# zoj613/OccuSpytial

Hardware: AMD Instinct MI355X
Metric: Gibbs iterations/sec on 100x100 ICAR lattice, 4 chains; 1/2/4/8 GPUs (higher is better)
Workload: dtype f64; 1 GPU; 100x100 queen ICAR lattice, 10000 sites, 5 visits/site, p=q=2, 4 chains per GPU batched in every kernel (BASELINE configs[1] data, the metric's 4 chains); chains_per_gpu=4, total_chains=4, sites=10000, visit_rows=50000, parallelism=chains sharded 4/GPU, no data-path collective; one GPU, communicator=single process, problem_transport=none, krylov_cap=0, stalls=0, solve_form=k_iter, one XCD per chain, solve_workgroups_per_chain=23, main_stream_cus=160, fused_fallbacks=0, threads_per_block=64

## Files before the change

occuspytial_amd/csrc/occ_kernels.hpp:

```cpp
#pragma once
#include <float.h>
#include <hip/hip_runtime.h>
#include <stdint.h>

#include "occ_plan.hpp"
#include "occ_rng.hpp"
#include "occ_state.hpp"

namespace occ {


#ifndef OCC_SLOT_ALIGN
#define OCC_SLOT_ALIGN 8
#endif
struct alignas(OCC_SLOT_ALIGN) Slot {
    double beta1, beta, oldb, alfa, dbar, epsln, phibar, rhs1, rhs2, tnorm2, gmax, gmin, cs, sn, root;
    double ibeta;
    int itn;
    int istop;
    int done;
    int pad;
};

#define OCC_SLOT_FIELDS(X) \
// ... 450 lines not shown
    for (int k = 0; k < D; ++k) {
        const double e = normal(k);
#pragma unroll
        for (int i = k; i < D; ++i) o[i] += U[k][i] * e;
    }
#pragma unroll
    for (int i = 0; i < D; ++i) o[i] += r[i];
#pragma unroll
    for (int i = 0; i < D; ++i) {
        double v = o[i];
#pragma unroll
        for (int k = 0; k < i; ++k) v -= U[k][i] * o[k];
        o[i] = v / U[i][i];
    }
#pragma unroll
    for (int i = D - 1; i >= 0; --i) {
        double v = o[i];
#pragma unroll
        for (int k = i + 1; k < D; ++k) v -= U[i][k] * o[k];
        o[i] = v / U[i][i];
    }
#pragma unroll
    for (int i = 0; i < D; ++i) out[i] = o[i];
    return ok;
}

template <int D>
__device__ __forceinline__ bool precision_mvnorm_reg(const double (&acc)[nacc(D)], const double *prec0, const double *pbm,
                                                     uint64_t key, uint32_t it, uint32_t stream, double (&out)[D],
                                                     const double *eps_inj = nullptr)
{
    return precision_mvnorm_with<D>(acc, prec0, pbm, out,
                                    [=](int k) { return eps_inj ? eps_inj[k] : block_normal(key, (uint32_t)k, 0, it, stream); });
}


enum : int { SYNC_MAIN = 0, SYNC_ALPHA = 16, SYNC_NOISE = 32, SYNC_MAIN_SEQ = 48, SYNC_SIDE_SEQ = 52, SYNC_ABORT = 56, SYNC_DEBUG = 57, SYNC_WORDS = 64 };
constexpr unsigned SYNC_SPIN_LIMIT = 1u << 19;

__device__ __forceinline__ unsigned sync_read(const unsigned *p)
{
    return __hip_atomic_load(p, __ATOMIC_RELAXED, __HIP_MEMORY_SCOPE_AGENT);
}
__device__ __forceinline__ void sync_set(unsigned *p, unsigned v)
{
    __hip_atomic_store(p, v, __ATOMIC_RELAXED, __HIP_MEMORY_SCOPE_AGENT);
}
__device__ __forceinline__ bool sync_wait(unsigned *sync, int word, unsigned target)
{
    unsigned spins = 0;
    while ((int)(sync_read(sync + word) - target) < 0) {
        __builtin_amdgcn_s_sleep(4);
        ++spins;
        if ((spins & 63u) == 0u && sync_read(sync + SYNC_ABORT) != 0u) return false;
        if (spins > SYNC_SPIN_LIMIT) {
            sync_set(sync + SYNC_ABORT, 1u);
            return false;
        }
    }
    return true;
}
__device__ __forceinline__ double load_agent(const double *p)
{
    return __hip_atomic_load(p, __ATOMIC_RELAXED, __HIP_MEMORY_SCOPE_AGENT);
}
__device__ __forceinline__ uint64_t uniform_u64(uint64_t v)
{
    const unsigned lo = (unsigned)__builtin_amdgcn_readfirstlane((int)(unsigned)v), hi = (unsigned)__builtin_amdgcn_readfirstlane((int)(unsigned)(v >> 32));
    return ((uint64_t)hi << 32) | lo;
}
__device__ __forceinline__ double uniform_f64(double v) { return __longlong_as_double((long long)uniform_u64((uint64_t)__double_as_longlong(v))); }

__global__ void __launch_bounds__(64) k_stream_probe_wait(unsigned *w)
{
    if (threadIdx.x != 0) return;
    unsigned seen = 0u, spins = 0u;
    for (; spins < (1u << 13); ++spins) {
        if (sync_read(w) != 0u) { seen = 1u; break; }
        __builtin_amdgcn_s_sleep(16);
    }
    w[16] = seen;
    w[17] = spins;
}
__global__ void __launch_bounds__(64) k_stream_probe_set(unsigned *w)
{
    if (threadIdx.x == 0) sync_set(w, 1u);
}

__global__ void __launch_bounds__(256) k_checksum(const unsigned char *__restrict__ data, unsigned long long bytes, unsigned long long *__restrict__ out)
{
    const unsigned long long nw = (bytes + 7ull) / 8ull;
    unsigned long long acc = 0ull;
    for (unsigned long long i = (unsigned long long)blockIdx.x * blockDim.x + threadIdx.x; i < nw; i += (unsigned long long)gridDim.x * blockDim.x) {
        unsigned long long w = 0ull;
        if (8ull * i + 8ull <= bytes) w = *reinterpret_cast<const unsigned long long *>(data + 8ull * i);
        else
            for (unsigned long long b = 8ull * i; b < bytes; ++b) w |= (unsigned long long)data[b] << (8ull * (b - 8ull * i));
        unsigned long long x = w + 0x9E3779B97F4A7C15ull * (i + 1ull);
        x = (x ^ (x >> 30)) * 0xBF58476D1CE4E5B9ull;
        x = (x ^ (x >> 27)) * 0x94D049BB133111EBull;
        acc += x ^ (x >> 31);
    }
    atomicAdd(out, acc);
}

__global__ void __launch_bounds__(256) k_snapshot(const double *__restrict__ eta, double *__restrict__ s_eta, const uint8_t *__restrict__ z, uint8_t *__restrict__ s_z,
                                                  const double2 *__restrict__ x, double2 *__restrict__ s_x, unsigned long long count,
                                                  const double *__restrict__ theta, double *__restrict__ s_theta, unsigned long long count_theta,
                                                  unsigned long long *__restrict__ clock,
                                                  ChainScalars *__restrict__ scs, int n_chains, int parity, uint32_t n_iter, uint32_t burnin, uint32_t keep)
{
    if (clock != nullptr && blockIdx.x == 0 && threadIdx.x < 4) clock[threadIdx.x] = threadIdx.x == 0 ? ~0ull : 0ull;
    if (scs != nullptr && blockIdx.x == 0) {
        for (int ch = (int)threadIdx.x; ch < n_chains; ch += (int)blockDim.x) {
            ChainScalars &sc = scs[ch];
            Ctl &ctl = sc.ctl[parity];
            sc.it_base = ctl.it;
            sc.it_stop = ctl.it + n_iter;
            sc.burnin = burnin;
            sc.keep = keep;
            ctl.koff = 0;
        }
    }
    for (unsigned long long i = (unsigned long long)blockIdx.x * blockDim.x + threadIdx.x; i < count; i += (unsigned long long)gridDim.x * blockDim.x) {
        s_eta[i] = eta[i];
        s_z[i] = z[i];
        s_x[i] = x[i];
    }
    for (unsigned long long i = (unsigned long long)blockIdx.x * blockDim.x + threadIdx.x; i < count_theta; i += (unsigned long long)gridDim.x * blockDim.x) s_theta[i] = theta[i];
}

__global__ void __launch_bounds__(64) k_gate(const Ctx *__restrict__ cp, ChainScalars *__restrict__ scs)
{
    const Ctx &c = *cp;
    if (c.sync == nullptr || threadIdx.x != 0) return;
    const unsigned j = c.sync[SYNC_SIDE_SEQ];
    if (c.sync[SYNC_DEBUG] != 0u) return;
    sync_set(c.sync + SYNC_NOISE, j);
    if (!sync_wait(c.sync, SYNC_MAIN, j)) scs[0].err = -2;
}

#define OCC_KARGS const Ctx *__restrict__ cp, ChainScalars *__restrict__ scs, Slot *__restrict__ slots, int chain_base, int e

__device__ __forceinline__ double quad_site(const Ctx &c, const double *eta, int i, double eta_i)
{
    const int lane = i & 63;
    int base, width;
    slice_of(c, i, base, width);
    double qe = c.qdiag[i] * eta_i;
    for (int k = 0; k < width; ++k) qe = fma(c.sell_val[base + k * 64 + lane], eta[c.sell_col[base + k * 64 + lane]], qe);
    return eta_i * qe;
}

template <int P>
__device__ __forceinline__ void omega_b_body(const Ctx &c, uint64_t key, const double (&beta)[P], int chain, uint32_t it, int blk,
                                             bool per_wave = false)
{
    const int n = c.n;
    const double *eta = c.eta + (size_t)chain * n;
    double om = 0.0;
    {
        const int i = blk * blockDim.x + threadIdx.x;
        if (i < n) {
            double xb = 0.0;
#pragma unroll
            for (int a = 0; a < P; ++a) xb += c.Xt[(size_t)a * n + i] * beta[a];
            om = pg1_draw(key, (uint32_t)i, it, STREAM_OMEGA_B, xb + eta[i]);
        }
    }
    int t = (int)threadIdx.x;
    asm volatile("" : "+v"(t));
    const int i = blk * (int)blockDim.x + t;
    double quad[1] = {0.0};
    if (i < n) {
        c.omega_b[it & 1][(size_t)chain * n + i] = om;
        quad[0] = quad_site(c, eta, i, eta[i]);
    }
    if (per_wave) {
        const double t = wave_sum(quad[0]);
        const int slice = blk * (int)(blockDim.x >> 6) + (int)(threadIdx.x >> 6);
        if ((threadIdx.x & 63) == 0 && slice < c.nb_n) c.part_quad[(size_t)chain * c.nb_n + slice] = t;
        return;
    }
    block_partials<1>(quad, c.part_quad + (size_t)chain * c.nb_n, c.nb_n, blk);
}

__device__ __forceinline__ void omega_b_body_g(const Ctx &c, const ChainScalars &sc, int chain, uint32_t it, int blk, bool per_wave = false)
{
    const int n = c.n, i = blk * blockDim.x + threadIdx.x;
    double quad[1] = {0.0};
    if (i < n) {
        const size_t ci = (size_t)chain * n + i;
        const double *eta = c.eta + (size_t)chain * n;
        double xb = 0.0;
        for (int a = 0; a < c.p; ++a) xb += c.Xt[(size_t)a * n + i] * sc.beta[a];
        const double eta_i = eta[i];
        c.omega_b[it & 1][ci] = pg1_draw(sc.key, (uint32_t)i, it, STREAM_OMEGA_B, xb + eta_i);
        quad[0] = quad_site(c, eta, i, eta_i);
    }
    if (per_wave) {
        const double t = wave_sum(quad[0]);
        const int slice = blk * (int)(blockDim.x >> 6) + (int)(threadIdx.x >> 6);
        if ((threadIdx.x & 63) == 0 && slice < c.nb_n) c.part_quad[(size_t)chain * c.nb_n + slice] = t;
        return;
    }
    block_partials<1>(quad, c.part_quad + (size_t)chain * c.nb_n, c.nb_n, blk);
}

template <int P>
__global__ void __launch_bounds__(256) k_omega_b(OCC_KARGS)
{
    const Ctx &c = *cp;
    const Tile tile = tile_of_block(chain_base);
    const int chain = tile.chain, blk = tile.blk;
    const ChainScalars &sc = scs[chain];
    const Ctl ctl = sc.ctl[e];
    if (ctl.koff || ctl.it >= sc.it_stop || sc.err != 0) return;
    if constexpr (P == 0) {
        omega_b_body_g(c, sc, chain, ctl.it, blk);
    } else {
        double beta[P];
#pragma unroll
        for (int a = 0; a < P; ++a) beta[a] = sc.beta[a];
        omega_b_body<P>(c, sc.key, beta, chain, ctl.it, blk);
    }
}

__global__ void __launch_bounds__(256) k_quad(OCC_KARGS)
{
    const Ctx &c = *cp;
    const Tile tile = tile_of_block(chain_base);
    const int chain = tile.chain, blk = tile.blk;
    const int n = c.n, i = blk * blockDim.x + threadIdx.x;
    const double *eta = c.eta + (size_t)chain * n;
    double quad[1] = {0.0};
    if (i < n) quad[0] = quad_site(c, eta, i, eta[i]);
    block_partials<1>(quad, c.part_quad + (size_t)chain * c.nb_n, c.nb_n, blk);
}

__device__ __forceinline__ void noise_site(const Ctx &c, uint64_t key, int chain, int i, uint32_t it)
{
    const int n = c.n, lane = i & 63;
    int base, width;
    slice_of(c, i, base, width);
    if (c.dense_F != nullptr) width = 0;
    double u = 0.0;
    for (int k = 0; k < width; ++k) {
        const int j = c.sell_col[base + k * 64 + lane];
        const double w = -c.sell_val[base + k * 64 + lane];
        if (w > 0.0) {
            const uint32_t lo = (uint32_t)min(i, j), hi = (uint32_t)max(i, j);
            const double t = sqrt(w) * block_normal(key, lo, hi, it, STREAM_ETA_EDGE);
            u += (i < j) ? t : -t;
        }
    }
    const size_t ci = (size_t)chain * n + i;
    if (c.dense_F == nullptr) c.uprior[it & 1][ci] = u;
    else if (i < c.dense_m) c.dense_eps[it & 1][(size_t)chain * c.dense_m + i] = block_normal(key, (uint32_t)i, 0, it, STREAM_ETA_DENSE);
    c.enorm[it & 1][ci] = block_normal(key, (uint32_t)i, 0, it, STREAM_ETA_SITE);
}

template <int NCH>
__global__ void __launch_bounds__(256) k_prior_dense(const Ctx *__restrict__ cp, ChainScalars *__restrict__ scs, int chain0, int e, int ahead)
{
    const Ctx &c = *cp;
    const int row = blockIdx.x * 4 + (int)(threadIdx.x >> 6), lane = threadIdx.x & 63;
    if (row >= c.n) return;
    const int m = c.dense_m;
    uint32_t it[NCH];
    bool on[NCH];
    bool any = false;
#pragma unroll
    for (int q = 0; q < NCH; ++q) {
        const int ch = chain0 + q;
        on[q] = false;
        it[q] = 0;
        if (ch < c.C) {
            const ChainScalars &sc = scs[ch];
            const Ctl ctl = sc.ctl[e];
            on[q] = !(ctl.koff || ctl.it >= sc.it_stop || sc.err != 0);
            it[q] = ctl.it + (uint32_t)ahead;
        }
        any = any || on[q];
    }
    if (!any) return;
    const double *F = c.dense_F + (size_t)row * m;
    double acc[NCH];
#pragma unroll
    for (int q = 0; q < NCH; ++q) acc[q] = 0.0;
    for (int j = lane; j < m; j += 64) {
        const double f = F[j];
#pragma unroll
        for (int q = 0; q < NCH; ++q)
            if (on[q]) acc[q] = fma(f, c.dense_eps[it[q] & 1][(size_t)(chain0 + q) * m + j], acc[q]);
    }
#pragma unroll
    for (int q = 0; q < NCH; ++q) {
        const double t = wave_sum(acc[q]);
        if (on[q] && lane == 0) c.uprior[it[q] & 1][(size_t)(chain0 + q) * c.n + row] = t;
    }
}

__global__ void __launch_bounds__(256) k_noise(OCC_KARGS, int ahead, int sync_on)
{
    __shared__ double s_red[NACC_G], s_U[MAXG * MAXG], s_work[2 * MAXG], s_alpha[MAXG];
    const Ctx &c = *cp;
    const Tile tile = tile_of_block_shared(c, 2, (c.n + (int)blockDim.x - 1) / (int)blockDim.x, chain_base);
    const int chain = tile.chain, blk = tile.blk;
    const bool synced = sync_on && c.sync;
    if (synced && blockIdx.x == 0 && blockIdx.y == 0 && threadIdx.x == 0) {
        const unsigned j = c.sync[SYNC_SIDE_SEQ];
        c.sync[SYNC_SIDE_SEQ] = j + 1u;
    }
    if (chain < 0) return;
    ChainScalars &sc = scs[chain];
    const Ctl ctl = sc.ctl[e];
    const bool idle = ctl.koff || ctl.it >= sc.it_stop || sc.err != 0;
    if (ahead == 1 && blk == 0) {
        if (!idle) {
            const int Q = c.q;
            reduce_partials_lds(c.part_alpha + (size_t)chain * nacc(Q) * c.nb_r, nacc(Q), c.nb_r, s_red);
            if (threadIdx.x == 0) {
                const double *a_prec = c.hyp, *a_pbm = c.hyp + Q * Q;
                const bool ok = precision_mvnorm_dev(Q, s_red, a_prec, a_pbm, sc.key, ctl.it, STREAM_ALPHA, s_U, s_work, s_alpha, nullptr);
                if (!ok) sc.err = -4;
                for (int a = 0; a < Q; ++a) __hip_atomic_store(&sc.alpha[a], s_alpha[a], __ATOMIC_RELAXED, __HIP_MEMORY_SCOPE_AGENT);
            }
        }
        if (synced && threadIdx.x == 0) {
            asm volatile("s_waitcnt vmcnt(0)" ::: "memory");
            __hip_atomic_fetch_add(c.sync + SYNC_ALPHA, 1u, __ATOMIC_RELAXED, __HIP_MEMORY_SCOPE_AGENT);
        }
    }
    if (idle) return;
    const uint32_t it_for = ctl.it + (uint32_t)ahead;
    if (blk == 0 && threadIdx.x == 0) {
        Cursor g(sc.key, 0u, it_for, STREAM_TAU);
        sc.tau_gamma[it_for & 1] = std_gamma(g, c.tau_shape);
    }
    if (blk == 0 && threadIdx.x >= 64 && (int)threadIdx.x - 64 < c.p) {
        const uint32_t k = threadIdx.x - 64u;
        sc.beta_eps[it_for & 1][k] = block_normal(sc.key, k, 0, it_for, STREAM_BETA);
    }
    const int i = blk * blockDim.x + threadIdx.x;
    if (i >= c.n) return;
    noise_site(c, sc.key, chain, i, it_for);
}

template <int INJ>
__global__ void __launch_bounds__(256) k_eta_init(OCC_KARGS)
{
    __builtin_amdgcn_s_setprio(3);
    const Ctx &c = *cp;
    const Tile tile = tile_of_block(chain_base);
    const int chain = tile.chain, blk = tile.blk;
    ChainScalars &sc = scs[chain];
    const Ctl ctl = sc.ctl[e];
    if (ctl.koff || ctl.it >= sc.it_stop || sc.err != 0) return;
    const int n = c.n, i = blk * blockDim.x + threadIdx.x;
// ... 1045 lines not shown
    double pr = num1, E = 0.0;
    int y_obs = 0, y_rep = 0, zi = 1;
    if (!not_surveyed) {
        double prod = 1.0, ll = seen ? lsig_e(a0, e0) : 0.0;
        const int r0 = c.site_ptr[sidx], r1 = c.site_ptr[sidx + 1];
        for (int r = r0; r < r1; ++r) {
            const double wa = wa_of(r), e = exp(-fabs(wa));
            const double d = expit_e(-wa, e);
            const double ur = block_uniform(key, (uint32_t)r, 0, it, STREAM_PPC);
            E += d;
            y_rep += (ur < d) ? 1 : 0;
            if (seen) {
                const int y = c.yrow[r] ? 1 : 0;
                y_obs += y;
                if (ll_on) ll += lsig_e(y ? -wa : wa, e);
            } else {
                const double ex = expit_e(wa, e);
                prod = (r == r0) ? ex : prod * ex;
            }
        }
        if (seen) {
            if (stats_on) site_add(c, chain, i, num1, 1.0, 1.0, eta_i);
            if (ll_on) ll_add(c, chain, i, exp(ll), ll);
        } else {
            const double num = num1 * prod;
            const double den = (1.0 - num1) + num;
            pr = num / den;
            if (ll_on) ll_add(c, chain, i, den, log(den));
        }
    }
    if (!seen) {
        const double u = block_uniform(key, (uint32_t)i, 0, it, STREAM_Z);
        zi = (u < pr) ? 1 : 0;
        c.z[(size_t)chain * n + i] = (uint8_t)zi;
        if (stats_on) site_add(c, chain, i, num1, pr, zi ? 1.0 : 0.0, eta_i);
    }
    if (!not_surveyed && zi) {
        const double se = sqrt(E), da = sqrt((double)y_obs) - se, db = sqrt((double)y_rep) - se;
        term[PPC_T_OBS] = ppc_fx(da * da);
        term[PPC_T_REP] = ppc_fx(db * db);
        term[PPC_DET_REP] = (unsigned long long)y_rep;
        term[PPC_SITES_REP] = y_rep > 0 ? 1ull : 0ull;
    }
    return zi;
}


template <int P, int STATS = 0>
__device__ __forceinline__ void z_ob_body(const Ctx &c, ChainScalars *__restrict__ scs, int chain_base, int e, bool synced, unsigned seq,
                                          bool per_wave, int debug_skip = 0,
                                          bool beta_ready = false)
{
    __shared__ int s_wait_ok, s_beta_ok;
    __shared__ double s_beta[P];
    const Tile tile = tile_of_block_shared(c, 0, 2 * (per_wave ? (c.n + (int)blockDim.x - 1) / (int)blockDim.x : c.nb_n), chain_base);
    const int chain = tile.chain, blk = tile.blk;
    if (chain < 0) return;
    ChainScalars &sc = scs[chain];
    constexpr int NQB = nacc(P);
    const bool draws = per_wave && !beta_ready && threadIdx.x < 64;
    const double *part_b = c.part_beta + (size_t)chain * NQB * c.nb_n;
    constexpr bool SUMS_PRE = P <= 4, EPS_PRE = P <= 2;
    double pre[PartialRounds<NQB>::R][NQB], eps2[2][P];
    if (draws) {
        if constexpr (SUMS_PRE) partials_load<NQB>(part_b, c.nb_n, 0, pre);
        if constexpr (EPS_PRE) {
#pragma unroll
            for (int h = 0; h < 2; ++h)
#pragma unroll
                for (int a = 0; a < P; ++a) eps2[h][a] = load_agent(&sc.beta_eps[h][a]);
        }
    }
    const uint64_t key = uniform_u64(sc.key);
    const Ctl ctl = sc.mid[e];
    const uint32_t it_stop = sc.it_stop;
    const int err0 = sc.err;
    asm volatile("" ::"s"(ctl.it), "s"(ctl.koff), "s"(it_stop), "s"(err0));
    const bool skip = ctl.koff || ctl.it >= it_stop || err0 != 0;
    const int nb = per_wave ? (c.n + (int)blockDim.x - 1) / (int)blockDim.x : c.nb_n;
    const uint32_t it = ctl.it;
    const bool writer = (blk == 0 && threadIdx.x == 0);
    if (writer) {
        Ctl nx = ctl;
        if (!skip) nx.it = it + 1;
        sc.ctl[e ^ 1] = nx;
        if (chain == chain_base && c.iter_clock != nullptr && c.iter_clock[1] != 0ull) {
            c.iter_clock[2] += c.iter_clock[1] - c.iter_clock[0];
            c.iter_clock[3] += 1ull;
            c.iter_clock[0] = ~0ull;
            c.iter_clock[1] = 0ull;
        }
        if (chain == chain_base && synced) c.sync[SYNC_MAIN_SEQ + (e ^ 1)] = seq + 1u;
        if (c.claim != nullptr) {
#pragma unroll
            for (int x = 0; x < 8; ++x) c.claim[(size_t)chain * 16 + x] = 0u;
        }
    }
    if (skip) return;
    double beta[P];
    if (beta_ready) {
#pragma unroll
        for (int a = 0; a < P; ++a) beta[a] = sc.beta[a];
    } else {
        double sums[NQB];
        if (!per_wave || !SUMS_PRE) reduce_partials<NQB>(part_b, c.nb_n, sums);
        else if (draws) {
#pragma unroll
            for (int r = 0; r < PartialRounds<NQB>::R; ++r)
#pragma unroll
                for (int qi = 0; qi < NQB; ++qi) asm volatile("" : "+v"(pre[r][qi]));
            if constexpr (EPS_PRE) {
#pragma unroll
                for (int h = 0; h < 2; ++h)
#pragma unroll
                    for (int a = 0; a < P; ++a) asm volatile("" : "+v"(eps2[h][a]));
            }
            reduce_partials_wave<NQB, true>(part_b, c.nb_n, pre, sums);
        }
        const double *b_prec = c.hyp + c.q * c.q + c.q, *b_pbm = b_prec + P * P;
        bool ok = true;
        if (!per_wave || threadIdx.x < 64) {
            if (EPS_PRE && per_wave) {
                ok = precision_mvnorm_with<P>(sums, b_prec, b_pbm, beta, [&](int k) {
                    const double odd = eps2[1][k], even = eps2[0][k];
                    return (it & 1u) ? odd : even;
                });
            } else {
                const double *eps = sc.beta_eps[it & 1];
                ok = precision_mvnorm_with<P>(sums, b_prec, b_pbm, beta, [=](int k) { return load_agent(eps + k); });
            }
            if (per_wave && threadIdx.x == 0) {
                s_beta_ok = ok ? 1 : 0;
#pragma unroll
                for (int a = 0; a < P; ++a) s_beta[a] = beta[a];
            }
        }
        if (per_wave) {
            __syncthreads();
            ok = s_beta_ok != 0;
#pragma unroll
            for (int a = 0; a < P; ++a) beta[a] = s_beta[a];
        }
        if (writer) {
            if (!ok) sc.err = -4;
#pragma unroll
            for (int a = 0; a < P; ++a) sc.beta[a] = beta[a];
        }
    }
    (void)nb;
#pragma unroll
    for (int a = 0; a < P; ++a) beta[a] = uniform_f64(beta[a]);
    if (blk & 1) {
        if (debug_skip & 2) return;
        omega_b_body<P>(c, key, beta, chain, it + 1u, blk >> 1, per_wave);
        return;
    }
    const int Q = c.q;
    double alpha[MAXC];
    if (synced) {
        if (threadIdx.x == 0) s_wait_ok = sync_wait(c.sync, SYNC_ALPHA, (seq + 1u) * (unsigned)c.C) ? 1 : 0;
        __syncthreads();
        if (!s_wait_ok && writer) sc.err = -2;
#pragma unroll
        for (int a = 0; a < MAXC; ++a) alpha[a] = (a < Q) ? load_agent(&sc.alpha[a]) : 0.0;
    } else {
#pragma unroll
        for (int a = 0; a < MAXC; ++a) alpha[a] = (a < Q) ? sc.alpha[a] : 0.0;
    }
    if (writer) record_draws<P>(c, sc, chain, it, alpha, beta, sc.tau);
    const int n = c.n, i = (blk >> 1) * blockDim.x + threadIdx.x;
    if constexpr (STATS == 4) {
        const uint32_t on = sc.site_on;
        const bool kept = it - sc.it_base >= sc.burnin, stats_on = (on & OUT_SITE) && kept, ll_on = (on & OUT_LL) && kept;
        if (debug_skip & 1) return;
        if (writer && stats_on) c.site_count[chain] += 1.0;
        if (writer && ll_on) c.ll_count[chain] += 1.0;
        uint32_t *row = region_row(c, sc, chain, it);
        unsigned long long *prow = ppc_row(c, sc, chain, it);
        const int g = (row != nullptr && i < n) ? (int)c.region_id[i] : -1;
        int zi = 0;
        unsigned long long term[PPC_NCOL] = {0ull, 0ull, 0ull, 0ull};
        if (i < n) {
            const double eta_i = c.eta[(size_t)chain * n + i];
            if (prow != nullptr) {
                zi = z_update_site_ppc(
                    c, key, chain, i, it, eta_i, stats_on, ll_on,
                    [&]() {
                        double xb = 0.0;
#pragma unroll
                        for (int a = 0; a < P; ++a) xb = fma(c.Xt[(size_t)a * c.n + i], beta[a], xb);
                        return xb;
                    },
                    [&](int r) {
                        double wa = 0.0;
#pragma unroll
                        for (int a = 0; a < MAXC; ++a)
                            if (a < c.q) wa = fma(c.Wt[(size_t)a * c.R + r], -alpha[a], wa);
                        return wa;
                    },
                    term);
            } else {
                zi = z_update_site<P, 0, 3>(c, key, chain, i, it, beta, alpha, eta_i, stats_on, ll_on);
            }
        }
        if (row != nullptr) region_count(row, c.region_G, g, zi);
        if (prow != nullptr) ppc_count(prow, term);
    } else if constexpr (STATS == 3) {
        const uint32_t on = sc.site_on;
        const bool kept = it - sc.it_base >= sc.burnin, stats_on = (on & OUT_SITE) && kept, ll_on = (on & OUT_LL) && kept;
        if (debug_skip & 1) return;
        if (writer && stats_on) c.site_count[chain] += 1.0;
        if (writer && ll_on) c.ll_count[chain] += 1.0;
        uint32_t *row = region_row(c, sc, chain, it);
        const int g = (row != nullptr && i < n) ? (int)c.region_id[i] : -1;
        int zi = 0;
        if (i < n) zi = z_update_site<P, 0, 3>(c, key, chain, i, it, beta, alpha, c.eta[(size_t)chain * n + i], stats_on, ll_on);
        if (row != nullptr) region_count(row, c.region_G, g, zi);
    } else if constexpr (STATS == 2) {
        const uint32_t on = sc.site_on;
        const bool kept = it - sc.it_base >= sc.burnin, stats_on = (on & OUT_SITE) && kept, ll_on = (on & OUT_LL) && kept;
        if (writer && stats_on && !(debug_skip & 1)) c.site_count[chain] += 1.0;
        if (writer && ll_on && !(debug_skip & 1)) c.ll_count[chain] += 1.0;
        if (i >= n || (debug_skip & 1)) return;
        z_update_site<P, 0, 2>(c, key, chain, i, it, beta, alpha, c.eta[(size_t)chain * n + i], stats_on, ll_on);
    } else if constexpr (STATS) {
        const bool stats_on = sc.site_on != 0u && it - sc.it_base >= sc.burnin;
        if (writer && stats_on && !(debug_skip & 1)) c.site_count[chain] += 1.0;
        if (i >= n || (debug_skip & 1)) return;
        z_update_site<P, 0, 1>(c, key, chain, i, it, beta, alpha, c.eta[(size_t)chain * n + i], stats_on);
    } else {
    if (i >= n || (debug_skip & 1)) return;
    z_update_site<P>(c, key, chain, i, it, beta, alpha, c.eta[(size_t)chain * n + i]);
    }
}

template <int INJ, int STATS = 0>
__device__ __forceinline__ int z_update_site_g(const Ctx &c, const ChainScalars &sc, int chain, int i, uint32_t it, double eta_i,
                                                bool stats_on = false, bool ll_on = false)
{
    if constexpr (STATS >= 2) {
        if (ll_on) {
            return z_update_site_ll<INJ>(
                c, sc.key, chain, i, it, eta_i, stats_on,
                [&]() {
                    double xb = 0.0;
                    for (int a = 0; a < c.p; ++a) xb = fma(c.Xt[(size_t)a * c.n + i], sc.beta[a], xb);
                    return xb;
                },
                [&](int r) {
                    double wa = 0.0;
                    for (int a = 0; a < c.q; ++a) wa = fma(c.Wt[(size_t)a * c.R + r], -sc.alpha[a], wa);
                    return wa;
                });
        }
    }
    const int sidx = c.site_sidx[i];
    const bool not_surveyed = sidx < 0;
    if (!not_surveyed && c.obs_site[sidx]) {
        if constexpr (STATS) {
            if (stats_on) {
                double xb = 0.0;
                for (int a = 0; a < c.p; ++a) xb = fma(c.Xt[(size_t)a * c.n + i], sc.beta[a], xb);
                site_add(c, chain, i, expit(xb + eta_i), 1.0, 1.0, eta_i);
            }
        }
        return 1;
    }
    const int n = c.n, P = c.p, Q = c.q;
    double xb = 0.0;
    for (int a = 0; a < P; ++a) xb = fma(c.Xt[(size_t)a * n + i], sc.beta[a], xb);
    const double num1 = expit(xb + eta_i);
    double pr = num1;
    if (!not_surveyed) {
        double prod = 1.0;
        const int r0 = c.site_ptr[sidx], r1 = c.site_ptr[sidx + 1];
        for (int r = r0; r < r1; ++r) {
            double wa = 0.0;
            for (int a = 0; a < Q; ++a) wa = fma(c.Wt[(size_t)a * c.R + r], -sc.alpha[a], wa);
            const double ex = expit(wa);
            prod = (r == r0) ? ex : prod * ex;
        }
        const double num = num1 * prod;
        pr = num / ((1.0 - num1) + num);
    }
    const double u = INJ ? c.inj->z_u[i] : block_uniform(sc.key, (uint32_t)i, 0, it, STREAM_Z);
    c.z[(size_t)chain * n + i] = (u < pr) ? 1 : 0;
    if constexpr (STATS) {
        if (stats_on) site_add(c, chain, i, num1, pr, (u < pr) ? 1.0 : 0.0, eta_i);
    }
    return (u < pr) ? 1 : 0;
}

template <int STATS = 0>
__device__ __forceinline__ void z_ob_body_g(const Ctx &c, ChainScalars *__restrict__ scs, int chain_base, int e, bool per_wave, int debug_skip)
{
    const Tile tile = tile_of_block(chain_base);
    const int chain = tile.chain, blk = tile.blk;
    ChainScalars &sc = scs[chain];
    const Ctl ctl = sc.mid[e];
    const bool skip = ctl.koff || ctl.it >= sc.it_stop || sc.err != 0;
    const uint32_t it = ctl.it;
    const bool writer = (blk == 0 && threadIdx.x == 0);
    if (writer) {
        Ctl nx = ctl;
        if (!skip) nx.it = it + 1;
        sc.ctl[e ^ 1] = nx;
    }
    if (skip) return;
    if (blk & 1) {
        if (debug_skip & 2) return;
        omega_b_body_g(c, sc, chain, it + 1u, blk >> 1, per_wave);
        return;
    }
    if (writer) {
        const uint32_t rel = it - sc.it_base;
        if (c.rec != nullptr && rel >= sc.burnin && rel - sc.burnin < sc.keep) {
            double *row = c.rec + ((size_t)chain * sc.keep + (rel - sc.burnin)) * (size_t)(c.q + c.p + 1);
            for (int a = 0; a < c.q; ++a) row[a] = sc.alpha[a];
            for (int a = 0; a < c.p; ++a) row[c.q + a] = sc.beta[a];
            row[c.q + c.p] = sc.tau;
        }
    }
    const int n = c.n, i = (blk >> 1) * blockDim.x + threadIdx.x;
    if constexpr (STATS == 4) {
        const uint32_t on = sc.site_on;
        const bool kept = it - sc.it_base >= sc.burnin, stats_on = (on & OUT_SITE) && kept, ll_on = (on & OUT_LL) && kept;
        if (debug_skip & 1) return;
        if (writer && stats_on) c.site_count[chain] += 1.0;
        if (writer && ll_on) c.ll_count[chain] += 1.0;
        uint32_t *row = region_row(c, sc, chain, it);
        unsigned long long *prow = ppc_row(c, sc, chain, it);
        const int g = (row != nullptr && i < n) ? (int)c.region_id[i] : -1;
        int zi = 0;
        unsigned long long term[PPC_NCOL] = {0ull, 0ull, 0ull, 0ull};
        if (i < n) {
            const double eta_i = c.eta[(size_t)chain * n + i];
            if (prow != nullptr) {
                zi = z_update_site_ppc(
                    c, uniform_u64(sc.key), chain, i, it, eta_i, stats_on, ll_on,
                    [&]() {
                        double xb = 0.0;
                        for (int a = 0; a < c.p; ++a) xb = fma(c.Xt[(size_t)a * c.n + i], sc.beta[a], xb);
                        return xb;
                    },
                    [&](int r) {
                        double wa = 0.0;
                        for (int a = 0; a < c.q; ++a) wa = fma(c.Wt[(size_t)a * c.R + r], -sc.alpha[a], wa);
                        return wa;
                    },
                    term);
            } else {
                zi = z_update_site_g<0, 3>(c, sc, chain, i, it, eta_i, stats_on, ll_on);
            }
        }
        if (row != nullptr) region_count(row, c.region_G, g, zi);
        if (prow != nullptr) ppc_count(prow, term);
    } else if constexpr (STATS == 3) {
        const uint32_t on = sc.site_on;
        const bool kept = it - sc.it_base >= sc.burnin, stats_on = (on & OUT_SITE) && kept, ll_on = (on & OUT_LL) && kept;
        if (debug_skip & 1) return;
        if (writer && stats_on) c.site_count[chain] += 1.0;
        if (writer && ll_on) c.ll_count[chain] += 1.0;
        uint32_t *row = region_row(c, sc, chain, it);
        const int g = (row != nullptr && i < n) ? (int)c.region_id[i] : -1;
        int zi = 0;
        if (i < n) zi = z_update_site_g<0, 3>(c, sc, chain, i, it, c.eta[(size_t)chain * n + i], stats_on, ll_on);
        if (row != nullptr) region_count(row, c.region_G, g, zi);
    } else if constexpr (STATS == 2) {
        const uint32_t on = sc.site_on;
        const bool kept = it - sc.it_base >= sc.burnin, stats_on = (on & OUT_SITE) && kept, ll_on = (on & OUT_LL) && kept;
        if (writer && stats_on && !(debug_skip & 1)) c.site_count[chain] += 1.0;
        if (writer && ll_on && !(debug_skip & 1)) c.ll_count[chain] += 1.0;
        if (i >= n || (debug_skip & 1)) return;
        z_update_site_g<0, 2>(c, sc, chain, i, it, c.eta[(size_t)chain * n + i], stats_on, ll_on);
    } else if constexpr (STATS) {
        const bool stats_on = sc.site_on != 0u && it - sc.it_base >= sc.burnin;
        if (writer && stats_on && !(debug_skip & 1)) c.site_count[chain] += 1.0;
        if (i >= n || (debug_skip & 1)) return;
        z_update_site_g<0, 1>(c, sc, chain, i, it, c.eta[(size_t)chain * n + i], stats_on);
    } else {
    if (i >= n || (debug_skip & 1)) return;
    z_update_site_g<0>(c, sc, chain, i, it, c.eta[(size_t)chain * n + i]);
    }
}

template <int P, int INJ = 0>
__global__ void __launch_bounds__(256) k_beta_draw(OCC_KARGS)
{
    const Ctx &c = *cp;
    const int chain = chain_base + blockIdx.x;
    ChainScalars &sc = scs[chain];
    const Ctl ctl = INJ ? sc.ctl[e] : sc.mid[e];
    if (ctl.koff || ctl.it >= sc.it_stop || sc.err != 0) return;
    if constexpr (P == 0) {
        __shared__ double s_red[NACC_G], s_U[MAXG * MAXG], s_work[2 * MAXG];
        const int p = c.p;
        reduce_partials_lds(c.part_beta + (size_t)chain * nacc(p) * c.nb_n, nacc(p), c.nb_n, s_red);
        if (threadIdx.x == 0) {
            const double *b_prec = c.hyp + c.q * c.q + c.q, *b_pbm = b_prec + p * p;
            const bool ok = precision_mvnorm_dev(p, s_red, b_prec, b_pbm, sc.key, ctl.it, STREAM_BETA, s_U, s_work, sc.beta,
                                                 INJ ? c.inj->beta_eps : sc.beta_eps[ctl.it & 1]);
            if (!ok) sc.err = -4;
        }
        return;
    } else {
    double sums[nacc(P)], beta[P];
    reduce_partials<nacc(P)>(c.part_beta + (size_t)chain * nacc(P) * c.nb_n, c.nb_n, sums);
    const double *b_prec = c.hyp + c.q * c.q + c.q, *b_pbm = b_prec + P * P;
    const bool ok = precision_mvnorm_reg<P>(sums, b_prec, b_pbm, sc.key, ctl.it, STREAM_BETA, beta, INJ ? c.inj->beta_eps : sc.beta_eps[ctl.it & 1]);
    if (threadIdx.x == 0) {
        if (!ok) sc.err = -4;
#pragma unroll
        for (int a = 0; a < P; ++a) sc.beta[a] = beta[a];
    }
    }
}

template <int P>
__global__ void __launch_bounds__(256, 3) k_z_ob(OCC_KARGS, int flags)
{
    __builtin_amdgcn_s_setprio(3);
    const Ctx &c = *cp;
    if constexpr (P == 0) {
        z_ob_body_g(c, scs, chain_base, e, (flags & 2) != 0, (flags >> 3) & 3);
    } else {
        const bool synced = (flags & 1) && c.sync != nullptr;
        const unsigned seq = synced ? (unsigned)__builtin_amdgcn_readfirstlane((int)c.sync[SYNC_MAIN]) : 0u;
        z_ob_body<P>(c, scs, chain_base, e, synced, seq, (flags & 2) != 0, (flags >> 3) & 3, (flags & 4) != 0);
    }
}

template <int P>
__global__ void __launch_bounds__(256, 3) k_z_ob_stats(OCC_KARGS, int flags)
{
    __builtin_amdgcn_s_setprio(3);
    const Ctx &c = *cp;
    if constexpr (P == 0) {
        z_ob_body_g<1>(c, scs, chain_base, e, (flags & 2) != 0, (flags >> 3) & 3);
    } else {
        const bool synced = (flags & 1) && c.sync != nullptr;
        const unsigned seq = synced ? (unsigned)__builtin_amdgcn_readfirstlane((int)c.sync[SYNC_MAIN]) : 0u;
        z_ob_body<P, 1>(c, scs, chain_base, e, synced, seq, (flags & 2) != 0, (flags >> 3) & 3, (flags & 4) != 0);
    }
}

template <int P>
__global__ void __launch_bounds__(256, 3) k_z_ob_ll(OCC_KARGS, int flags)
{
    __builtin_amdgcn_s_setprio(3);
    const Ctx &c = *cp;
    if constexpr (P == 0) {
        z_ob_body_g<2>(c, scs, chain_base, e, (flags & 2) != 0, (flags >> 3) & 3);
    } else {
        const bool synced = (flags & 1) && c.sync != nullptr;
        const unsigned seq = synced ? (unsigned)__builtin_amdgcn_readfirstlane((int)c.sync[SYNC_MAIN]) : 0u;
        z_ob_body<P, 2>(c, scs, chain_base, e, synced, seq, (flags & 2) != 0, (flags >> 3) & 3, (flags & 4) != 0);
    }
}

template <int P>
__global__ void __launch_bounds__(256, 3) k_z_ob_occ(OCC_KARGS, int flags)
{
    __builtin_amdgcn_s_setprio(3);
    const Ctx &c = *cp;
    if constexpr (P == 0) {
        z_ob_body_g<3>(c, scs, chain_base, e, (flags & 2) != 0, (flags >> 3) & 3);
    } else {
        const bool synced = (flags & 1) && c.sync != nullptr;
        const unsigned seq = synced ? (unsigned)__builtin_amdgcn_readfirstlane((int)c.sync[SYNC_MAIN]) : 0u;
        z_ob_body<P, 3>(c, scs, chain_base, e, synced, seq, (flags & 2) != 0, (flags >> 3) & 3, (flags & 4) != 0);
    }
}

template <int P>
__global__ void __launch_bounds__(256, 3) k_z_ob_ppc(OCC_KARGS, int flags)
{
    __builtin_amdgcn_s_setprio(3);
    const Ctx &c = *cp;
    if constexpr (P == 0) {
        z_ob_body_g<4>(c, scs, chain_base, e, (flags & 2) != 0, (flags >> 3) & 3);
    } else {
        const bool synced = (flags & 1) && c.sync != nullptr;
        const unsigned seq = synced ? (unsigned)__builtin_amdgcn_readfirstlane((int)c.sync[SYNC_MAIN]) : 0u;
        z_ob_body<P, 4>(c, scs, chain_base, e, synced, seq, (flags & 2) != 0, (flags >> 3) & 3, (flags & 4) != 0);
    }
}

template <int P>
__global__ void __launch_bounds__(256) k_cond_beta_z(OCC_KARGS)
{
    const Ctx &c = *cp;
    const Tile tile = tile_of_block(chain_base);
    const int chain = tile.chain, blk = tile.blk;
    ChainScalars &sc = scs[chain];
    const Inject &inj = *c.inj;
    const Ctl ctl = sc.ctl[e];
    if constexpr (P == 0) {
        const int n = c.n, i = blk * blockDim.x + threadIdx.x;
        if (inj.do_z && i < n) z_update_site_g<1>(c, sc, chain, i, ctl.it, c.eta[(size_t)chain * n + i]);
        return;
    } else {
    double beta[P];
    if (inj.do_beta) {
        double sums[nacc(P)];
        reduce_partials<nacc(P)>(c.part_beta + (size_t)chain * nacc(P) * c.nb_n, c.nb_n, sums);
        const double *b_prec = c.hyp + c.q * c.q + c.q, *b_pbm = b_prec + P * P;
        const bool ok = precision_mvnorm_reg<P>(sums, b_prec, b_pbm, sc.key, ctl.it, STREAM_BETA, beta, inj.beta_eps);
        if (blk == 0 && threadIdx.x == 0) {
            if (!ok) sc.err = -4;
#pragma unroll
            for (int a = 0; a < P; ++a) sc.beta[a] = beta[a];
        }
    } else {
#pragma unroll
        for (int a = 0; a < P; ++a) beta[a] = sc.beta[a];
    }
    if (!inj.do_z) return;
    double alpha[MAXC];
#pragma unroll
    for (int a = 0; a < MAXC; ++a) alpha[a] = (a < c.q) ? sc.alpha[a] : 0.0;
    const int n = c.n, i = blk * blockDim.x + threadIdx.x;
    if (i < n) z_update_site<P, 1>(c, sc.key, chain, i, ctl.it, beta, alpha, c.eta[(size_t)chain * n + i]);
    }
}

enum : int { DRAW_PG1 = 0, DRAW_STD_GAMMA = 1, DRAW_NORMAL = 2, DRAW_UNIFORM = 3, DRAW_WAVE_SUM_CHECK = 4 };
__global__ void __launch_bounds__(256) k_draw(int kind, uint64_t key, uint32_t it, uint32_t stream, long long n, const double *__restrict__ param,
                                              double *__restrict__ out)
{
    const long long i = (long long)blockIdx.x * blockDim.x + threadIdx.x;
    if (kind == DRAW_WAVE_SUM_CHECK) {
        double x[4], y[4], z[4];
#pragma unroll
        for (int q = 0; q < 4; ++q) {
            x[q] = (i < n) ? param[i] * (1.0 + 0.37 * q) + (q == 3 ? param[i] * param[i] : 0.0) : 0.0;
            y[q] = x[q];
// ... 25 lines not shown
```

Baseline: 79570 iterations/s.

## Move ICAR quadratic form from omega-b blocks to z-update blocks with prefetch

In the fused beta/z/omega kernel, the per-site ICAR quadratic-form term is no longer computed by the odd (omega_b) blocks. The even (z-update) blocks now compute it instead. They issue the SELL column, value and neighbour-eta loads for up to 8 neighbours before the alpha sync wait and z update, then finish the FMA chain afterwards. This hides gather latency behind the sync and z work and rebalances load between the two block types. In exchange it keeps about 16 extra doubles live per thread, which raises register pressure and may lower occupancy. Out-of-range threads are clamped to the last site, so they also issue loads.

```diff
diff --git a/occuspytial_amd/csrc/occ_kernels.hpp b/occuspytial_amd/csrc/occ_kernels.hpp
--- a/occuspytial_amd/csrc/occ_kernels.hpp
+++ b/occuspytial_amd/csrc/occ_kernels.hpp
@@ -626,7 +626,56 @@
     return eta_i * qe;
 }
 
-template <int P>
+constexpr int QUAD_WIN = 8;
+struct QuadPre {
+    double qd, eta_i, val[QUAD_WIN], eta_j[QUAD_WIN];
+    int col[QUAD_WIN], base, width, lane, ic;
+};
+__device__ __forceinline__ void quad_load_site(const Ctx &c, int i, QuadPre &q)
+{
+    const int ic = min(i, c.n - 1);
+    q.ic = ic;
+    q.lane = ic & 63;
+    slice_of(c, ic, q.base, q.width);
+#pragma unroll
+    for (int k = 0; k < QUAD_WIN; ++k) q.col[k] = c.sell_col[q.base + ((k < q.width) ? k * 64 : 0) + q.lane];
+}
+__device__ __forceinline__ void quad_load_neighbours(const Ctx &c, const double *eta, QuadPre &q)
+{
+    q.qd = c.qdiag[q.ic];
+    q.eta_i = eta[q.ic];
+#pragma unroll
+    for (int k = 0; k < QUAD_WIN; ++k) {
+        q.val[k] = c.sell_val[q.base + ((k < q.width) ? k * 64 : 0) + q.lane];
+        q.eta_j[k] = eta[q.col[k]];
+    }
+}
+__device__ __forceinline__ double quad_finish(const Ctx &c, const double *eta, QuadPre &q)
+{
+#pragma unroll
+    for (int k = 0; k < QUAD_WIN; ++k) asm volatile("" : "+v"(q.val[k]), "+v"(q.eta_j[k]));
+    double qe = q.qd * q.eta_i;
+#pragma unroll
+    for (int k = 0; k < QUAD_WIN; ++k) {
+        const double t = fma(q.val[k], q.eta_j[k], qe);
+        qe = (k < q.width) ? t : qe;
+    }
+    for (int k = QUAD_WIN; k < q.width; ++k) qe = fma(c.sell_val[q.base + k * 64 + q.lane], eta[c.sell_col[q.base + k * 64 + q.lane]], qe);
+    return q.eta_i * qe;
+}
+__device__ __forceinline__ void quad_store(const Ctx &c, int chain, int blk, bool per_wave, double site_term)
+{
+    double quad[1] = {site_term};
+    if (per_wave) {
+        const double t = wave_sum(quad[0]);
+        const int slice = blk * (int)(blockDim.x >> 6) + (int)(threadIdx.x >> 6);
+        if ((threadIdx.x & 63) == 0 && slice < c.nb_n) c.part_quad[(size_t)chain * c.nb_n + slice] = t;
+        return;
+    }
+    block_partials<1>(quad, c.part_quad + (size_t)chain * c.nb_n, c.nb_n, blk);
+}
+
+template <int P, bool QUAD = true>
 __device__ __forceinline__ void omega_b_body(const Ctx &c, uint64_t key, const double (&beta)[P], int chain, uint32_t it, int blk,
                                              bool per_wave = false)
 {
@@ -645,24 +694,19 @@
     int t = (int)threadIdx.x;
     asm volatile("" : "+v"(t));
     const int i = blk * (int)blockDim.x + t;
-    double quad[1] = {0.0};
+    double quad = 0.0;
     if (i < n) {
         c.omega_b[it & 1][(size_t)chain * n + i] = om;
-        quad[0] = quad_site(c, eta, i, eta[i]);
-    }
-    if (per_wave) {
-        const double t = wave_sum(quad[0]);
-        const int slice = blk * (int)(blockDim.x >> 6) + (int)(threadIdx.x >> 6);
-        if ((threadIdx.x & 63) == 0 && slice < c.nb_n) c.part_quad[(size_t)chain * c.nb_n + slice] = t;
-        return;
-    }
-    block_partials<1>(quad, c.part_quad + (size_t)chain * c.nb_n, c.nb_n, blk);
-}
-
+        if constexpr (QUAD) quad = quad_site(c, eta, i, eta[i]);
+    }
+    if constexpr (QUAD) quad_store(c, chain, blk, per_wave, quad);
+}
+
+template <bool QUAD = true>
 __device__ __forceinline__ void omega_b_body_g(const Ctx &c, const ChainScalars &sc, int chain, uint32_t it, int blk, bool per_wave = false)
 {
     const int n = c.n, i = blk * blockDim.x + threadIdx.x;
-    double quad[1] = {0.0};
+    double quad = 0.0;
     if (i < n) {
         const size_t ci = (size_t)chain * n + i;
         const double *eta = c.eta + (size_t)chain * n;
@@ -670,15 +714,9 @@
         for (int a = 0; a < c.p; ++a) xb += c.Xt[(size_t)a * n + i] * sc.beta[a];
         const double eta_i = eta[i];
         c.omega_b[it & 1][ci] = pg1_draw(sc.key, (uint32_t)i, it, STREAM_OMEGA_B, xb + eta_i);
-        quad[0] = quad_site(c, eta, i, eta_i);
-    }
-    if (per_wave) {
-        const double t = wave_sum(quad[0]);
-        const int slice = blk * (int)(blockDim.x >> 6) + (int)(threadIdx.x >> 6);
-        if ((threadIdx.x & 63) == 0 && slice < c.nb_n) c.part_quad[(size_t)chain * c.nb_n + slice] = t;
-        return;
-    }
-    block_partials<1>(quad, c.part_quad + (size_t)chain * c.nb_n, c.nb_n, blk);
+        if constexpr (QUAD) quad = quad_site(c, eta, i, eta_i);
+    }
+    if constexpr (QUAD) quad_store(c, chain, blk, per_wave, quad);
 }
 
 template <int P>
@@ -2030,9 +2068,13 @@
     for (int a = 0; a < P; ++a) beta[a] = uniform_f64(beta[a]);
     if (blk & 1) {
         if (debug_skip & 2) return;
-        omega_b_body<P>(c, key, beta, chain, it + 1u, blk >> 1, per_wave);
+        omega_b_body<P, false>(c, key, beta, chain, it + 1u, blk >> 1, per_wave);
         return;
     }
+    const double *eta_ch = c.eta + (size_t)chain * c.n;
+    QuadPre qp;
+    quad_load_site(c, (blk >> 1) * (int)blockDim.x + (int)threadIdx.x, qp);
+    quad_load_neighbours(c, eta_ch, qp);
     const int Q = c.q;
     double alpha[MAXC];
     if (synced) {
@@ -2047,6 +2089,7 @@
     }
     if (writer) record_draws<P>(c, sc, chain, it, alpha, beta, sc.tau);
     const int n = c.n, i = (blk >> 1) * blockDim.x + threadIdx.x;
+    auto z_part = [&]() {
     if constexpr (STATS == 4) {
         const uint32_t on = sc.site_on;
         const bool kept = it - sc.it_base >= sc.burnin, stats_on = (on & OUT_SITE) && kept, ll_on = (on & OUT_LL) && kept;
@@ -2110,6 +2153,10 @@
     if (i >= n || (debug_skip & 1)) return;
     z_update_site<P>(c, key, chain, i, it, beta, alpha, c.eta[(size_t)chain * n + i]);
     }
+    };
+    z_part();
+    const double term = quad_finish(c, eta_ch, qp);
+    quad_store(c, chain, blk >> 1, per_wave, i < n ? term : 0.0);
 }
 
 template <int INJ, int STATS = 0>
@@ -2187,7 +2234,7 @@
     if (skip) return;
     if (blk & 1) {
         if (debug_skip & 2) return;
-        omega_b_body_g(c, sc, chain, it + 1u, blk >> 1, per_wave);
+        omega_b_body_g<false>(c, sc, chain, it + 1u, blk >> 1, per_wave);
         return;
     }
     if (writer) {
@@ -2200,6 +2247,11 @@
         }
     }
     const int n = c.n, i = (blk >> 1) * blockDim.x + threadIdx.x;
+    const double *eta_ch = c.eta + (size_t)chain * n;
+    QuadPre qp;
+    quad_load_site(c, i, qp);
+    quad_load_neighbours(c, eta_ch, qp);
+    auto z_part = [&]() {
     if constexpr (STATS == 4) {
         const uint32_t on = sc.site_on;
         const bool kept = it - sc.it_base >= sc.burnin, stats_on = (on & OUT_SITE) && kept, ll_on = (on & OUT_LL) && kept;
@@ -2260,6 +2312,10 @@
     if (i >= n || (debug_skip & 1)) return;
     z_update_site_g<0>(c, sc, chain, i, it, c.eta[(size_t)chain * n + i]);
     }
+    };
+    z_part();
+    const double term = quad_finish(c, eta_ch, qp);
+    quad_store(c, chain, blk >> 1, per_wave, i < n ? term : 0.0);
 }
 
 template <int P, int INJ = 0>
```

Result: no change. 79450 iterations/s (-0.2%).
